# songhayeong/aes-fhe

Hardware: AMD Instinct MI355X
Metric: AES-128 blocks/sec (homomorphic full round) at N=2^16, L=30; 1/2/4/8 MI355X (higher is better)
Workload: dtype u64

## Files before the change

aes-fhe_amd/csrc/bconv_cols.h:

```cpp
#pragma once
#include "bconv_mfma.h"
#include "ntt256f.h"

namespace aesfhe {

__device__ __forceinline__ void cols256_stages_store(double (&x)[16], double q, double qi, bool big, const double* tg,
                                                     const double* tws, double* s, u64* out, int b, int cl, int c) {
#pragma unroll
    for (int st = 0; st < 4; st++) {
        const int m = 1 << st, hh = 8 >> st;
        if (big && st == 2) {
#pragma unroll
            for (int a = 0; a < 16; a++) x[a] = fred(x[a], q, qi);
        }
#pragma unroll
        for (int a = 0; a < 16; a++) {
            if (a & hh) continue;
            const int ti = m + (a >> (4 - st));
            ct_f(x[a], x[a + hh], tg[ti], q, qi);
        }
    }
#pragma unroll
    for (int a = 0; a < 16; a++) s[(a * 16 + b) * kPadF + cl] = x[a];
    __syncthreads();
// ... 6 lines not shown
        if (big && (st & 1) == 0) {
#pragma unroll
            for (int bb = 0; bb < 16; bb++) x[bb] = fred(x[bb], q, qi);
        }
#pragma unroll
        for (int bb = 0; bb < 16; bb++) {
            if (bb & hh) continue;
            ct_f(x[bb], x[bb + hh], tws[m + ap * (m >> 4) + (bb >> (8 - st))], q, qi);
        }
    }
#pragma unroll
    for (int bb = 0; bb < 16; bb++) st_d(&out[(ap * 16 + bb) * 256 + c], x[bb]);
}

template <int NSTEP, bool YIN, bool VC = false, int PF = 1, int TT = 4, int LT = 2, int MODE = 0>
__global__ __launch_bounds__(256, TT == 4 ? 2 : 3) void k_bconv_cols(BconvArgs a, Tabs T, int ntile) {
    static_assert(TT == 4 || TT == 2, "4 or 2 targets per workgroup");
    static_assert(LT == 1 || LT == 2, "1 or 2 LDS tiles");
    __shared__ double s[LT][256 * kPadF];
    __shared__ double tws[TT][256];
    const int tid = threadIdx.x, lane = tid & 63, w = tid >> 6, c = lane & 31, h = lane >> 5;
    const int cl = tid & 15, b = tid >> 4;
    const int id = blockIdx.x, x8 = id & 7, j = id >> 3;
    const int tile = j % ntile, u = (j / ntile) * 8 + x8;
    const int bx = u & 15, z = u >> 4, zb = z / a.nc, zc = z - zb * a.nc;
    const int logN = T.logN;
    const u64* src = a.src + (long)zb * a.sbs + (long)zc * a.scs;
    u64* dst = a.dst + (long)zb * a.dbs + (long)zc * a.dcs;
    auto limb_of = [&](int tau) { return tau < a.skip0 ? tau : tau + a.skipn; };
    auto pid_of = [&](int tl) { return tl <= a.tl_l ? tl : a.Lp1 + tl - a.tl_l - 1; };
    const int tau0 = TT * tile;
    const int nlive = min(TT, a.nt - tau0);
#pragma unroll
    for (int m = 0; m < TT; m++)
        if (m < nlive) tws[m][tid] = T.psid[((long)pid_of(limb_of(tau0 + m)) << logN) + tid];
    bc_v4i af[NSTEP];
    {
        const int row = lane & 31, ta = row >> 3, pb = (row & 3) + 4 * ((row >> 2) & 1);
        const int tau = tau0 + ta;
        const bc_v4i* ap =
            (const bc_v4i*)(a.tab + ((long)(ta < TT && tau < a.nt ? pid_of(limb_of(tau)) : 0) * 8 + pb) * kBconvKT + 16 * h);
#pragma unroll
        for (int st = 0; st < NSTEP; st++) af[st] = ap[2 * st];
    }
    const u64* sp[NSTEP][2];
    double sq[NSTEP][2], sf[NSTEP][2];
#pragma unroll
    for (int st = 0; st < NSTEP; st++)
#pragma unroll
        for (int uu = 0; uu < 2; uu++) {
            const int sl = 4 * st + 2 * h + uu;
            const int i = sl < a.ns ? sl : 0;
            sp[st][uu] = src + ((long)i << logN) + bx * 16 + (c & 15);
            if (!YIN) {
                const int pid = i < a.s_nq ? a.s_q0 + i : a.s_p0 + i - a.s_nq;
                sq[st][uu] = (double)a.qall[pid];
                sf[st][uu] = a.sinvf[i];
            }
        }
    double xv[TT][16];
    double eq[TT], eqi[TT], ew32[TT], ef32[TT], ecr[TT];
#pragma unroll
    for (int m = 0; m < TT; m++) {
        const int pid = tau0 + m < a.nt ? pid_of(limb_of(tau0 + m)) : 0;
        const double* pc = a.pc + 4 * pid;
        eq[m] = pc[0], eqi[m] = pc[1], ew32[m] = pc[2], ef32[m] = pc[3], ecr[m] = a.corr[pid];
    }
    double ev[VC ? 4 * NSTEP : 1];
#pragma unroll
    for (int sl = 0; sl < (VC ? 4 * NSTEP : 0); sl++) ev[sl] = a.einv[sl];
    u64 raw[PF + 1][NSTEP][2][2];
    auto load = [&](u64 (&r)[NSTEP][2][2], int ar) {
#pragma unroll
        for (int st = 0; st < NSTEP; st++)
#pragma unroll
            for (int uu = 0; uu < 2; uu++)
#pragma unroll
                for (int g = 0; g < 2; g++) r[st][uu][g] = sp[st][uu][(16 * ar + 4 * w + 2 * g + (c >> 4)) * 256];
    };
#pragma unroll
    for (int p = 0; p < PF; p++) load(raw[p], p);
#pragma unroll
    for (int ar = 0; ar < 16; ar++) {
        if (ar + PF < 16) load(raw[(ar + PF) % (PF + 1)], ar + PF);
        bc_v4i bf[2][NSTEP];
        double ys[2][NSTEP][2];
#pragma unroll
        for (int st = 0; st < NSTEP; st++)
#pragma unroll
            for (int uu = 0; uu < 2; uu++)
#pragma unroll
                for (int g = 0; g < 2; g++) {
                    u64 yb = PF ? raw[ar % (PF + 1)][st][uu][g] : sp[st][uu][(16 * ar + 4 * w + 2 * g + (c >> 4)) * 256];
                    if (!YIN) {
                        const double q = sq[st][uu], f = sf[st][uu];
                        double y = fmul_rem(u2d(yb), tw_w(f, q), f, q);
                        y = y < 0.0 ? y + q : y;
                        yb = (u64)__double_as_longlong(y + 4503599627370496.0) & 0xFFFFFFFFFFFFFULL;
                    }
                    if (VC) ys[g][st][uu] = u2d(yb);
                    bf[g][st][2 * uu] = (int)(unsigned)yb ^ (int)0x80808080;
                    bf[g][st][2 * uu + 1] = (int)(unsigned)(yb >> 32) ^ (int)0x80808080;
                }
        if constexpr (VC) {
            double yl[NSTEP][2][2];
#pragma unroll
            for (int st = 0; st < NSTEP; st++)
#pragma unroll
                for (int uu = 0; uu < 2; uu++) swap_halves(ys[0][st][uu], ys[1][st][uu], yl[st][uu][0], yl[st][uu][1]);
            double sum = 0.0;
#pragma unroll
            for (int st = 0; st < NSTEP; st++)
#pragma unroll
                for (int hh = 0; hh < 2; hh++)
#pragma unroll
                    for (int uu = 0; uu < 2; uu++) {
                        const int sl = 4 * st + 2 * hh + uu;
                        sum = sum + yl[st][uu][hh] * ev[sl];
                    }
            const int vown = (int)__builtin_rint(sum);
            const auto pr = __builtin_amdgcn_permlane32_swap((unsigned)vown, (unsigned)vown, false, false);
            const int voth = (int)(h ? pr[0] : pr[1]);
#pragma unroll
            for (int st = 0; st < NSTEP; st++)
#pragma unroll
                for (int uu = 0; uu < 2; uu++)
                    if (4 * st + 2 * h + uu == a.ns) {
#pragma unroll
                        for (int g = 0; g < 2; g++) {
                            bf[g][st][2 * uu] = ((g == h ? vown : voth) & 0xff) ^ (int)0x80808080;
                            bf[g][st][2 * uu + 1] = (int)0x80808080;
                        }
                    }
        }
        if constexpr (MODE == 2) {
#pragma unroll
            for (int m = 0; m < TT; m++) xv[m][ar] = (double)(bf[0][0][0] & 0xffffff) + (double)(bf[1][NSTEP - 1][3] & 0xff);
            continue;
        }
        bc_v16i acc[2];
#pragma unroll
        for (int g = 0; g < 2; g++) {
            acc[g] = bc_v16i{};
#pragma unroll
            for (int st = 0; st < NSTEP; st++) acc[g] = __builtin_amdgcn_mfma_i32_32x32x32_i8(af[st], bf[g][st], acc[g], 0, 0, 0);
        }
#pragma unroll
        for (int m = 0; m < TT; m++) {
            if (m >= nlive) break;
            double part[2];
#pragma unroll
            for (int g = 0; g < 2; g++) {
                const int p01 = acc[g][4 * m] + acc[g][4 * m + 1] * 256, p23 = acc[g][4 * m + 2] + acc[g][4 * m + 3] * 256;
                part[g] = __builtin_fma((double)p23, 65536.0, (double)p01);
            }
            double lo, hi;
            swap_halves(part[0], part[1], lo, hi);
            xv[m][ar] = fred(lo + fmul_rem(hi, ew32[m], ef32[m], eq[m]) + ecr[m], eq[m], eqi[m]);
        }
    }
    __syncthreads();
    if constexpr (MODE == 1) {
#pragma unroll
        for (int m = 0; m < TT; m++) {
            if (m >= nlive) break;
            u64* o = dst + ((long)limb_of(tau0 + m) << logN);
#pragma unroll
            for (int ar = 0; ar < 16; ar++) st_d(&o[(ar * 16 + b) * 256 + bx * 16 + cl], xv[m][ar]);
        }
        return;
    }
#pragma unroll
    for (int m = 0; m < TT; m++) {
        if (m >= nlive) break;
        if (LT == 1 && m > 0) __syncthreads();
        const int tl = limb_of(tau0 + m), pid = pid_of(tl);
        const double q = (double)T.q[pid], qi = T.qinv[pid];
        cols256_stages_store(xv[m], q, qi, q >= kBigPrime, T.psid + ((long)pid << logN), tws[m], s[m % LT],
                             dst + ((long)tl << logN), b, cl, bx * 16 + cl);
    }
}

}
```

aes-fhe_amd/csrc/bconv_mfma.h:

```cpp
#pragma once
#include "kernels.h"
#include "basis_tables.h"

namespace aesfhe {

typedef int bc_v4i __attribute__((ext_vector_type(4)));
typedef int bc_v16i __attribute__((ext_vector_type(16)));

struct BconvArgs {
    const u64* src;
    long sbs, scs;
    u64* dst;
    long dbs, dcs;
    int nc;
    int ns;
    int s_nq, s_q0, s_p0;
    const double* sinvf;
    const double* einv;
    int nt, skip0, skipn, tl_l, Lp1;
    const int8_t* tab;
    const double* corr;
    const double* pc;
    const u64* qall;
    const double* qinvall;
    int tiles_per_group;
};

__device__ __forceinline__ void swap_halves(double x, double y, double& xo, double& yo) {
    const u64 a = (u64)__double_as_longlong(x), b = (u64)__double_as_longlong(y);
    const auto lo = __builtin_amdgcn_permlane32_swap((unsigned)a, (unsigned)b, false, false);
    const auto hi = __builtin_amdgcn_permlane32_swap((unsigned)(a >> 32), (unsigned)(b >> 32), false, false);
    xo = __longlong_as_double((long long)(((u64)(unsigned)hi[0] << 32) | (unsigned)lo[0]));
    yo = __longlong_as_double((long long)(((u64)(unsigned)hi[1] << 32) | (unsigned)lo[1]));
}

template <int NSTEP, bool VC>
__global__ __launch_bounds__(256, 3) void k_bconv_mfma(BconvArgs a, int logN) {
    const int lane = threadIdx.x & 63, w = threadIdx.x >> 6;
    const int c = lane & 31, h = lane >> 5;
    const int z = blockIdx.z, zb = z / a.nc, zc = z - zb * a.nc;
    const long kb = (long)blockIdx.x * 256 + w * 64;
    const u64* src = a.src + (long)zb * a.sbs + (long)zc * a.scs;
    bc_v4i bf[2][NSTEP];
    double ys[2][2 * NSTEP];
#pragma unroll
    for (int s = 0; s < NSTEP; s++) {
#pragma unroll
        for (int u = 0; u < 2; u++) {
            const int sl = 4 * s + 2 * h + u;
            const bool live = sl < a.ns;
            const int i = live ? sl : 0;
            const int pid = i < a.s_nq ? a.s_q0 + i : a.s_p0 + i - a.s_nq;
            const double q = (double)a.qall[pid];
            const double f = a.sinvf[i], wv = tw_w(f, q);
            const u64* sp = src + ((long)i << logN) + kb + c;
#pragma unroll
            for (int g = 0; g < 2; g++) {
                double y = fmul_rem(u2d(sp[32 * g]), wv, f, q);
                y = y < 0.0 ? y + q : y;
                ys[g][2 * s + u] = live ? y : 0.0;
                const u64 yb = live ? ((u64)__double_as_longlong(y + 4503599627370496.0) & 0xFFFFFFFFFFFFFULL) : 0;
                bf[g][s][2 * u] = (int)(unsigned)yb ^ (int)0x80808080;
                bf[g][s][2 * u + 1] = (int)(unsigned)(yb >> 32) ^ (int)0x80808080;
            }
        }
    }
    if constexpr (VC) {
#pragma unroll
        for (int g = 0; g < 2; g++) {
            double other[2 * NSTEP];
#pragma unroll
// ... 93 lines not shown
```

aes-fhe_amd/csrc/engine.hip:

```cpp
#include <hip/hip_runtime.h>

#include <algorithm>
#include <atomic>
#include <cstdarg>
#include <cstdlib>
#include <cstdio>
#include <cstring>
#include <map>
#include <unordered_map>
#include <memory>
#include <mutex>
#include <string>
#include <vector>

#include "../../include/aesfhe.h"
#include "kernels_ops.h"
#include "ntt256f.h"
#include "ks_fused.h"
#include "bconv_mfma.h"
#include "bconv_cols.h"
#include "basis_tables.h"
#include "bsgs_plan.h"
#include "operands.h"
#include "arena.h"
// ... 399 lines not shown
    o.ptr = v.zero ? nullptr : v.d;
    o.bs = bcast_stride(v.B, v.bs, outB);
    o.ps = v.ps;
    o.np = v.np;
    o.bmask = (v.B > 1 && v.B < outB) ? v.B - 1 : -1;
    return o;
}

static Out out_of(aesfhe_ct* c) {
    Out o;
    o.ptr = c->d;
    o.ps = (long)(c->level + 1) * c->eng->N;
    o.bs = (long)c->np * o.ps;
    return o;
}

static View view_of(const CtPtr& c) { return view_of(c.get()); }
static Out out_of(const CtPtr& c) { return out_of(c.get()); }

static dim3 ew_grid(aesfhe_engine* e, int y, int z) { return dim3(e->N / 256, y, z); }

template <int R1>
static void ntt_fwd_t(aesfhe_engine* e, Span src, Span dst, int total) {
    constexpr int CW = (kTile / R1) < kC2 ? (kTile / R1) : kC2;
    constexpr int RW = (kTile / kC2) < R1 ? (kTile / kC2) : R1;
    Tabs T = e->tabs();
    const double by = 8.0 * e->N * (double)total;
    {
        ProfScope ps(e, FAM_NTT, by, "ntt_generic");
        hipLaunchKernelGGL(k_ntt_fwd_cols<R1>, dim3(kC2 / CW, total), dim3(256), 0, e->stream, src, dst, T);
    }
    {
        ProfScope ps(e, FAM_NTT, by, "ntt_generic");
        hipLaunchKernelGGL(k_ntt_fwd_rows<R1>, dim3(R1 / RW, total), dim3(256), 0, e->stream, dst, T);
    }
}
template <int R1>
static void ntt_inv_t(aesfhe_engine* e, Span src, Span dst, int total) {
    constexpr int CW = (kTile / R1) < kC2 ? (kTile / R1) : kC2;
    constexpr int RW = (kTile / kC2) < R1 ? (kTile / kC2) : R1;
    Tabs T = e->tabs();
    const double by = 8.0 * e->N * (double)total;
    {
        ProfScope ps(e, FAM_NTT, by, "ntt_generic");
        hipLaunchKernelGGL(k_ntt_inv_rows<R1>, dim3(R1 / RW, total), dim3(256), 0, e->stream, src, dst, T);
    }
    {
        ProfScope ps(e, FAM_NTT, by, "ntt_generic");
        hipLaunchKernelGGL(k_ntt_inv_cols<R1>, dim3(kC2 / CW, total), dim3(256), 0, e->stream, dst, T);
    }
}

template <int R>
static void ntt256(aesfhe_engine* e, Span src, Span dst, int total, bool inverse, const double* lf = nullptr) {
    Tabs T = e->tabs();
    const double by = 8.0 * e->N * (double)total;
    {
        ProfScope ps(e, FAM_NTT, by, inverse ? "ntt_inv_rows" : "ntt_fwd_cols");
        if (!inverse) hipLaunchKernelGGL(k_nttf_fwd_cols<R>, dim3(16, total), dim3(256), 0, e->stream, src, dst, T);
        else hipLaunchKernelGGL((k_nttf_inv_rows<R, false>), dim3(R / 16, total), dim3(256), 0, e->stream, src, dst, T, Span{}, (const u64*)nullptr);
    }
    ProfScope ps(e, FAM_NTT, by, inverse ? "ntt_inv_cols" : "ntt_fwd_rows");
    if (!inverse) hipLaunchKernelGGL((k_nttf_fwd_rows_t<false, R>), dim3(R / 16, total), dim3(256), 0, e->stream, dst, T, RowFin{});
    else if (lf) hipLaunchKernelGGL((k_nttf_inv_cols<R, true>), dim3(16, total), dim3(256), 0, e->stream, dst, T, lf);
    else hipLaunchKernelGGL((k_nttf_inv_cols<R, false>), dim3(16, total), dim3(256), 0, e->stream, dst, T, (const double*)nullptr);
}

static bool fused_ntt(const aesfhe_engine* e) { return e->logN == 16 || e->logN == 17; }

static void intt_prod(aesfhe_engine* e, Span a, Span b, Span dst, int total, const u64* fac, const double* lf = nullptr) {
    if (total <= 0) return;
    Tabs T = e->tabs();
    const double by = 8.0 * e->N * (double)total;
    {
        ProfScope ps(e, FAM_NTT, 2.0 * by, "ntt_inv_rows_prod");
        if (e->logN == 16) {
            if (fac) hipLaunchKernelGGL((k_nttf_inv_rows<256, true, true>), dim3(16, total), dim3(256), 0, e->stream, a, dst, T, b, fac);
            else hipLaunchKernelGGL((k_nttf_inv_rows<256, true, false>), dim3(16, total), dim3(256), 0, e->stream, a, dst, T, b, fac);
        } else {
            if (fac) hipLaunchKernelGGL((k_nttf_inv_rows<512, true, true>), dim3(32, total), dim3(256), 0, e->stream, a, dst, T, b, fac);
            else hipLaunchKernelGGL((k_nttf_inv_rows<512, true, false>), dim3(32, total), dim3(256), 0, e->stream, a, dst, T, b, fac);
        }
    }
    ProfScope ps(e, FAM_NTT, by, "ntt_inv_cols");
    if (e->logN == 16) {
        if (lf) hipLaunchKernelGGL((k_nttf_inv_cols<256, true>), dim3(16, total), dim3(256), 0, e->stream, dst, T, lf);
        else hipLaunchKernelGGL((k_nttf_inv_cols<256, false>), dim3(16, total), dim3(256), 0, e->stream, dst, T, lf);
    } else {
        if (lf) throw_err(AESFHE_EUNSUPPORTED, "per-limb INTT factors at N = 2^17");
        hipLaunchKernelGGL((k_nttf_inv_cols<512, false>), dim3(16, total), dim3(256), 0, e->stream, dst, T, lf);
    }
    HIPC(hipGetLastError());
}

static void ntt_fwd_cols(aesfhe_engine* e, Span src, Span dst, int total) {
    if (e->logN == 16) hipLaunchKernelGGL(k_nttf_fwd_cols<256>, dim3(16, total), dim3(256), 0, e->stream, src, dst, e->tabs());
    else hipLaunchKernelGGL(k_nttf_fwd_cols<512>, dim3(16, total), dim3(256), 0, e->stream, src, dst, e->tabs());
}
static void ntt_fwd_cols(aesfhe_engine* e, Span sp, int total) { ntt_fwd_cols(e, sp, sp, total); }

static void ntt(aesfhe_engine* e, Span src, Span dst, int total, bool inverse) {
    if (total <= 0) return;
    if (e->logN == 16 || e->logN == 17) {
        if (e->logN == 16) ntt256<256>(e, src, dst, total, inverse);
        else ntt256<512>(e, src, dst, total, inverse);
        HIPC(hipGetLastError());
        return;
    }
    switch (e->logN) {
#define CASE(LG, R)                                                        \
    case LG:                                                               \
        if (inverse) ntt_inv_t<R>(e, src, dst, total);                     \
        else ntt_fwd_t<R>(e, src, dst, total);                             \
        break;
        CASE(10, 4)
        CASE(11, 8)
        CASE(12, 16)
        CASE(13, 32)
        CASE(14, 64)
        CASE(15, 128)
        CASE(16, 256)
        CASE(17, 512)
#undef CASE
        default:
            throw_err(AESFHE_EUNSUPPORTED, "log_n %d not supported by the HIP NTT", e->logN);
    }
    HIPC(hipGetLastError());
}

static Span span_s(u64* base, long pstride, int nl, int nq, int qpid0, int spid0) {
    Span s;
    s.base = base;
    s.pstride = pstride;
    s.nl = nl;
    s.nq = nq;
    s.qpid0 = qpid0;
    s.spid0 = spid0;
    return s;
}


static void build_tables(aesfhe_engine* e) {
    const int N = e->N, np = e->np, L = e->L, K = e->K, Lp1 = e->Lp1;
// ... 1204 lines not shown
    const dim3 g(N / 256, groups, nz);
#define BCV(S, V) hipLaunchKernelGGL((k_bconv_mfma<S, V>), g, dim3(256), 0, e->stream, a, e->logN)
    switch (nstep * 2 + (vc ? 1 : 0)) {
        case 2: BCV(1, false); break;
        case 3: BCV(1, true); break;
        case 4: BCV(2, false); break;
        case 5: BCV(2, true); break;
        case 6: BCV(3, false); break;
        case 7: BCV(3, true); break;
        case 8: BCV(4, false); break;
        default: BCV(4, true); break;
    }
#undef BCV
    HIPC(hipGetLastError());
}

static bool fused_bconv(const aesfhe_engine* e) { return e->logN == 16; }

static BconvArgs modup_args(const aesfhe_engine* e, const u64* dc, int l, int j, u64* dst, bool ysrc) {
    const int lo = j * e->A, alpha = std::min(lo + e->A, l + 1) - lo, ne = l + 1 + e->K;
    const size_t set = (size_t)j * e->A + (alpha - 1);
    BconvArgs a{};
    a.src = dc + (long)lo * e->N;
    a.sbs = (long)(l + 1) * e->N;
    a.dst = dst;
    a.dbs = (long)ne * e->N;
    a.nc = 1;
    a.ns = alpha;
    a.s_nq = alpha;
    a.s_q0 = lo;
    a.sinvf = ysrc ? nullptr : e->mu_hatinvf + set * e->A;
    a.nt = ne - alpha;
    a.skip0 = lo;
    a.skipn = alpha;
    a.tl_l = l;
    a.Lp1 = e->Lp1;
    a.tab = e->bc_mu_tab + set * e->np * 8 * kBconvKT;
    a.corr = e->bc_mu_corr + set * e->np;
    a.pc = e->bc_pc;
    a.qall = e->q;
    a.qinvall = e->qinv;
    return a;
}

static MdTabs md_tabs(const aesfhe_engine* e, int l, int r) {
    if (r < 0 || r > kMdrMaxR || e->K + r > kMdrMaxE || l - r < 0) throw_err(AESFHE_EARG, "bad combined rescale depth %d", r);
    const size_t cell = md_cell(e->Lp1, r, l), ce = cell * kMdrMaxE, cl = cell * e->Lp1;
    const MdTabs& b = e->md;
    return {b.invf + ce, b.ninvf + ce, b.einv + ce, b.tab + cl * kBconvRow, b.corr + cl,
            b.dinv + cl, b.dinvf + cl, b.hatf + cl * kMdrMaxE, b.dmodf + cl};
}

static BconvArgs moddown_args(const aesfhe_engine* e, const MdTabs& t, const u64* acc, long abs_, long acs, int l, int r,
                              u64* dst, bool ysrc) {
    const int lk = l - r;
    const long kN = (long)(lk + 1) * e->N;
    BconvArgs a{};
    a.src = acc + kN;
    a.sbs = abs_;
    a.scs = acs;
    a.dst = dst;
    a.dbs = 2 * kN;
    a.dcs = kN;
    a.nc = 2;
    a.ns = e->K + r;
    a.s_nq = r;
    a.s_q0 = lk + 1;
    a.s_p0 = e->Lp1;
    a.sinvf = ysrc ? nullptr : t.invf;
    a.einv = t.einv;
    a.nt = lk + 1;
    a.skip0 = lk + 1;
    a.skipn = 0;
    a.tl_l = lk;
    a.Lp1 = e->Lp1;
    a.tab = t.tab;
    a.corr = t.corr;
    a.pc = e->bc_pc;
    a.qall = e->q;
    a.qinvall = e->qinv;
    return a;
}

template <bool VC>
static void launch_bconv_cols_t(aesfhe_engine* e, const BconvArgs& a, int nz, int nslots) {
    const int nstep = (nslots + 3) / 4, ntile = (a.nt + 3) / 4;
    if (e->logN != 16 || nstep < 1 || nstep > 4 || ntile < 1 || (16 * nz) % 8)
        throw_err(AESFHE_EUNSUPPORTED, "fused base conversion of %d slots to %d targets", nslots, a.nt);
    if (!a.src || !a.dst || !a.tab || !a.corr || !a.pc || (VC && !a.einv))
        throw_err(AESFHE_EUNSUPPORTED, "fused base conversion with a missing table");
    const dim3 g((unsigned)(16 * nz * ntile));
    const Tabs T = e->tabs();
#define BCC(S) hipLaunchKernelGGL((k_bconv_cols<S, true, VC, 1>), g, dim3(256), 0, e->stream, a, T, ntile)
    switch (nstep) {
        case 1: BCC(1); break;
        case 2: BCC(2); break;
        case 3: BCC(3); break;
        default: BCC(4); break;
    }
#undef BCC
    HIPC(hipGetLastError());
}
static void launch_bconv_cols(aesfhe_engine* e, const BconvArgs& a, int nz) { launch_bconv_cols_t<false>(e, a, nz, a.ns); }

static std::vector<unsigned short> bsgs_block_order(int logN, const std::vector<u64>& gal) {
    std::vector<unsigned short> ord;
    if (!aesfhe::bsgs_block_order(logN, std::vector<uint64_t>(gal.begin(), gal.end()), ord))
        throw_err(AESFHE_EUNSUPPORTED, "bsgs block order is not a permutation");
    return ord;
}

static int ks_beta(const aesfhe_engine* e, int l) {
    const int beta = (l + 1 + e->A - 1) / e->A;
    if (beta > 12) throw_err(AESFHE_EUNSUPPORTED, "more than 12 key-switch digits");
    return beta;
}
static void check_key_digits(aesfhe_engine* e, const aesfhe_key* k, int l) {
    if (k && k->ndig > 0 && ks_beta(e, l) > k->ndig)
        throw_err(AESFHE_ELEVEL, "key trimmed to %d digits cannot switch at level %d (%d digits)", k->ndig, l, ks_beta(e, l));
}

static void ks_modup(aesfhe_engine* e, const u64* d, long dbs, int B, int l, u64* ext, bool cols_only = false,
                     const Opnd* pa = nullptr, const Opnd* pb = nullptr, const u64* fac = nullptr) {
    const int N = e->N, K = e->K, ne = l + 1 + K;
    const long lN = (long)(l + 1) * N, neN = (long)ne * N;
    const int beta = ks_beta(e, l);
    Tmp dc(e, (size_t)B * lN);
    const bool fcols = fused_bconv(e);
    const double* lf = fcols ? e->mu_nhatf + (size_t)l * e->Lp1 : nullptr;
    Span sdc = span_s(dc.p, lN, l + 1, l + 1, 0, e->Lp1);
    if (pa) {
        Span sa = span_s((u64*)pa->ptr + pa->ps, pa->bs, l + 1, l + 1, 0, e->Lp1);
        Span sb = span_s((u64*)pb->ptr + pb->ps, pb->bs, l + 1, l + 1, 0, e->Lp1);
        sa.pmask = pa->bmask;
        sb.pmask = pb->bmask;
        intt_prod(e, sa, sb, sdc, B * (l + 1), fac, lf);
    } else {
        Span sd = span_s((u64*)d, dbs, l + 1, l + 1, 0, e->Lp1);
        if (lf) ntt256<256>(e, sd, sdc, B * (l + 1), true, lf);
        else ntt(e, sd, sdc, B * (l + 1), true);
    }
    Tmp mu;
    bool any_wide = false;
    for (int j = 0; j < beta; j++) any_wide |= std::min((j + 1) * e->A, l + 1) - j * e->A > 1;
    if (cols_only && any_wide && !fcols) mu = Tmp(e, (size_t)B * neN);
    for (int j = 0; j < beta; j++) {
        const int A = e->A, lo = j * A, hi = std::min(lo + A, l + 1), alpha = hi - lo;
        u64* exj = ext + (size_t)j * B * neN;
        u64* muj = mu ? mu.p : exj;
        if (cols_only && alpha == 1) {
            const SpreadSrc ss{(const u64*)dc.p + (long)lo * N, lN, 0, 0, 0.0};
            auto kern = N == 65536 ? k_nttf_fwd_cols_spread<256, 3> : k_nttf_fwd_cols_spread<512, 3>;
            auto cols = [&](Span sp, int total) {
                ProfScope ps(e, FAM_NTT, 8.0 * N * (double)total, "ntt_fwd_cols_spread");
                hipLaunchKernelGGL(kern, dim3(16, total), dim3(256), 0, e->stream, ss, sp, e->tabs());
            };
            if (lo > 0) cols(span_s(exj, neN, lo, lo, 0, e->Lp1), B * lo);
            cols(span_s(exj + (long)hi * N, neN, ne - hi, (l + 1) - hi, hi, e->Lp1), B * (ne - hi));
            HIPC(hipGetLastError());
            continue;
        }
        if (fcols) {
            const BconvArgs a = modup_args(e, dc.p, l, j, exj, true);
            {
                ProfScope ps(e, FAM_KS, 8.0 * N * (double)B * ne, "modup_cols");
                launch_bconv_cols(e, a, B);
            }
            if (!cols_only) {
                auto rows = [&](long off, int n, int nq, int p0, int total) {
                    ProfScope ps(e, FAM_NTT, 8.0 * N * (double)total, "ntt_fwd_rows");
                    hipLaunchKernelGGL((k_nttf_fwd_rows_t<false, 256>), dim3(16, total), dim3(256), 0, e->stream,
                                       span_s(exj + off, neN, n, nq, p0, e->Lp1), e->tabs(), RowFin{});
                    HIPC(hipGetLastError());
                };
                if (lo > 0) rows(0, lo, lo, 0, B * lo);
                rows((long)hi * N, ne - hi, (l + 1) - hi, hi, B * (ne - hi));
            }
            continue;
        }
        {
            ProfScope ps(e, FAM_KS, 8.0 * N * (double)B * ne, "modup");
            launch_bconv(e, modup_args(e, dc.p, l, j, muj, false), B, alpha, false);
        }
        auto fwd = [&](long off, int n, int nq, int p0, int total) {
            Span sp = span_s(exj + off, neN, n, nq, p0, e->Lp1);
            if (!cols_only) return ntt(e, sp, sp, total, false);
            ProfScope ps(e, FAM_NTT, 8.0 * N * (double)total, "ntt_fwd_cols");
            ntt_fwd_cols(e, span_s(muj + off, neN, n, nq, p0, e->Lp1), sp, total);
        };
        if (lo > 0) fwd(0, lo, lo, 0, B * lo);
        fwd((long)hi * N, ne - hi, (l + 1) - hi, hi, B * (ne - hi));
    }
}

static void ks_inner_acc(aesfhe_engine* e, const u64* d, long dbs, const u64* ext, int B, int l,
                         const aesfhe_key* k, Opnd addend, bool pmod, u64* acc, bool ext_cols, bool accum = false) {
    const int N = e->N, K = e->K, ne = l + 1 + K;
    const long neN = (long)ne * N;
    const int beta = ks_beta(e, l);
    check_key_digits(e, k, l);
    const double* pm = pmod ? (const double*)e->pmodf : (const double*)nullptr;
    if (ext_cols) {
        const int nown = std::min(l + 1, beta * e->A);
        const double opw = (double)nown + (pmod && addend.ptr ? (double)addend.np * (l + 1) : 0.0);
        ProfScope ps(e, FAM_KS, 8.0 * N * ((double)B * (beta * ne - nown + opw) + (double)ne * (2.0 * beta + 2.0 * B * (accum ? 2 : 1))), "ks_rows_acc.ks");
        const int R = N / 256, blocks = 8 * B * (ne * (R / 8) / 8);
        const Opnd none{nullptr, 0, 0, 0};
        auto kern = R == 256 ? k_nttf_rows_ks<1, 256, false> : k_nttf_rows_ks<1, 512, false>;
        hipLaunchKernelGGL(kern, dim3(blocks), dim3(256), 0, e->stream, d, dbs, ext, neN, (long)B * neN, (const u64*)k->d, 2L * e->np * N, (long)e->np * N, acc, 2 * neN, neN, B, beta, e->A, l, ne, e->tabs(), addend, pm, (int)accum, none, (const u64*)nullptr, none, 0, ne, KsFin{});
    } else {
        ProfScope ps(e, FAM_KS, 8.0 * N * (double)ne * (beta * B + 2.0 * beta + 2.0 * B * (accum ? 2 : 1)), "ks_inner");
        auto inner = beta <= 4 ? k_ks_inner_all<4> : beta <= 8 ? k_ks_inner_all<8> : k_ks_inner_all<12>;
        hipLaunchKernelGGL(inner, dim3(N / 256, ne, 1), dim3(256), 0, e->stream, d, dbs, ext, neN, (long)B * neN, (const u64*)k->d, 2L * e->np * N, (long)e->np * N, acc, 2 * neN, neN, B, beta, e->A, l, e->q, e->qinv, e->Lp1, addend, pm, e->logN, (int)accum);
    }
    HIPC(hipGetLastError());
}

static void moddown_conv(aesfhe_engine* e, const MdTabs& t, u64* acc, long abs_, long acs, int B, int l, int r, u64* conv,
                         bool rows_done) {
    const int N = e->N, K = e->K, lk = l - r;
    const long kN = (long)(lk + 1) * N;
    {
        Span ssp = span_s(acc + kN, acs, K + r, r, lk + 1, e->Lp1);
        const int total = B * 2 * (K + r);
        if (rows_done) {
            ProfScope ps(e, FAM_NTT, 8.0 * N * (double)total, "ntt_inv_cols");
            if (N == 65536) hipLaunchKernelGGL((k_nttf_inv_cols<256, false>), dim3(16, total), dim3(256), 0, e->stream, ssp, e->tabs(), (const double*)nullptr);
            else hipLaunchKernelGGL((k_nttf_inv_cols<512, false>), dim3(16, total), dim3(256), 0, e->stream, ssp, e->tabs(), (const double*)nullptr);
            HIPC(hipGetLastError());
        } else {
            ntt(e, ssp, ssp, total, true);
        }
    }
    {
        ProfScope ps(e, FAM_KS, 8.0 * N * (double)B * 2 * (K + r + lk + 1), "moddown");
        if (K + r < 1 || K + r > 16) throw_err(AESFHE_EUNSUPPORTED, "ModDown source width outside 1..16");
        if (K + r + 1 <= 16)
            launch_bconv(e, moddown_args(e, t, acc, abs_, acs, l, r, conv, false), B * 2, K + r + 1, true);
        else
            AESFHE_DISPATCH16(K + r, launch_moddown, dim3(N / 512, bconv_groups(N, B * 2, lk + 1), B * 2), e->stream, (const u64*)acc, abs_, acs, l, r, conv, 2 * kN, kN,
                              t.invf, t.hatf, t.einv, t.dmodf, e->Lp1, e->q, e->qinv, e->logN, kMdrMaxE);
    }
    HIPC(hipGetLastError());
}

static bool moddown_cols_ok(const aesfhe_engine* e, int r) { return fused_bconv(e) && e->K + r + 1 <= 16; }
static void moddown_conv_cols(aesfhe_engine* e, const MdTabs& t, u64* acc, long abs_, long acs, int B, int l, int r,
                              u64* conv2, bool rows_done) {
    const int N = e->N, K = e->K, lk = l - r;
    {
        Span ssp = span_s(acc + (long)(lk + 1) * N, acs, K + r, r, lk + 1, e->Lp1);
        const int total = B * 2 * (K + r);
        if (!rows_done) {
            ProfScope ps(e, FAM_NTT, 8.0 * N * (double)total, "ntt_inv_rows");
            hipLaunchKernelGGL((k_nttf_inv_rows<256, false>), dim3(16, total), dim3(256), 0, e->stream, ssp, ssp, e->tabs(),
                               Span{}, (const u64*)nullptr);
            HIPC(hipGetLastError());
        }
        ProfScope ps(e, FAM_NTT, 8.0 * N * (double)total, "ntt_inv_cols");
        hipLaunchKernelGGL((k_nttf_inv_cols<256, true>), dim3(16, total), dim3(256), 0, e->stream, ssp, e->tabs(), t.ninvf);
        HIPC(hipGetLastError());
    }
    ProfScope ps(e, FAM_KS, 8.0 * N * (double)B * 2 * (K + r + lk + 1), "moddown_cols");
    launch_bconv_cols_t<true>(e, moddown_args(e, t, acc, abs_, acs, l, r, conv2, true), 2 * B, K + r + 1);
}

struct Conv2 {
    Tmp conv, buf;
};
template <typename F>
static Conv2 moddown_conv2(aesfhe_engine* e, const MdTabs& t, u64* acc, long abs_, long acs, int B, int l, int r,
                           bool rows_done, F converted) {
    const int lk = l - r, total = B * 2 * (lk + 1);
    const long kN = (long)(lk + 1) * e->N;
    Conv2 c;
    if (moddown_cols_ok(e, r)) {
        c.buf = Tmp(e, (size_t)B * 2 * kN);
        moddown_conv_cols(e, t, acc, abs_, acs, B, l, r, c.buf.p, rows_done);
        converted();
        return c;
    }
    c.conv = Tmp(e, (size_t)B * 2 * kN);
    moddown_conv(e, t, acc, abs_, acs, B, l, r, c.conv.p, rows_done);
    converted();
    c.buf = Tmp(e, (size_t)B * 2 * kN);
    ProfScope ps(e, FAM_NTT, 8.0 * e->N * (double)total, "ntt_fwd_cols");
    ntt_fwd_cols(e, span_s(c.conv.p, kN, lk + 1, lk + 1, 0, e->Lp1), span_s(c.buf.p, kN, lk + 1, lk + 1, 0, e->Lp1), total);
    return c;
}

static void moddown_acc(aesfhe_engine* e, u64* acc, int B, int l, int r, Opnd fin_add, aesfhe_ct* o) {
    const int N = e->N, ne = l + 1 + e->K, lk = l - r;
    const long neN = (long)ne * N, kN = (long)(lk + 1) * N;
    const MdTabs t = md_tabs(e, l, r);
    if (fused_ntt(e)) {
        const Conv2 c = moddown_conv2(e, t, acc, 2 * neN, neN, B, l, r, false, [] {});
        const int total = B * 2 * (lk + 1);
        RowFin f{(const u64*)acc, 2 * neN, neN, Opnd2{fin_add.ptr, fin_add.bs, fin_add.ps, fin_add.np}, o->d,
                 2 * kN, kN, t.dinvf, lk + 1};
        ProfScope ps(e, FAM_NTT, 8.0 * N * (double)total * (3.0 + (fin_add.ptr ? 1.0 : 0.0)), "ntt_fwd_rows_fin");
        auto kern = N == 65536 ? k_nttf_fwd_rows_t<true, 256> : k_nttf_fwd_rows_t<true, 512>;
        hipLaunchKernelGGL(kern, dim3(N / 4096, total), dim3(256), 0, e->stream, span_s(c.buf.p, kN, lk + 1, lk + 1, 0, e->Lp1),
                           e->tabs(), f);
        HIPC(hipGetLastError());
        return;
    }
    Tmp conv(e, (size_t)B * 2 * kN);
    moddown_conv(e, t, acc, 2 * neN, neN, B, l, r, conv.p, false);
    Span sc = span_s(conv.p, kN, lk + 1, lk + 1, 0, e->Lp1);
    ntt(e, sc, sc, B * 2 * (lk + 1), false);
    ProfScope psf(e, FAM_KS, 8.0 * N * (double)B * 2 * (lk + 1) * 4, "moddown_finish");
    hipLaunchKernelGGL(k_moddown_finish, dim3(N / 256, lk + 1, B * 2), dim3(256), 0, e->stream, (const u64*)acc, 2 * neN, neN, (const u64*)conv.p, 2 * kN, kN, fin_add, out_of(o), e->q, t.dinv, t.dinvf, e->logN);
    HIPC(hipGetLastError());
}

template <int R>
static decltype(&k_nttf_rows_ks_p<R, false, 1>) ks_rows_kernel(bool prod, bool fin) {
// ... 1090 lines not shown
```

aes-fhe_amd/csrc/ntt256f.h:

```cpp
#pragma once
#include <type_traits>

#include "kernels.h"

namespace aesfhe {


__device__ __forceinline__ void ct_f(double& x, double& y, double w, double q, double qi) {
    const double v = fmul_remq(y, w, qi, q);
    const double t = x;
    x = t + v;
    y = t - v;
}
template <bool FOLD>
__device__ __forceinline__ void gs_f(double& x, double& y, double w, double q, double qi) {
    const double s = x + y, d = x - y;
    x = FOLD ? fred(s, q, qi) : s;
    y = fmul_remq(d, w, qi, q);
}
__device__ __forceinline__ double tw_row(const double* W, int idx, double rw, double q, double qi) {
    return fmul_remq(W[idx], rw, qi, q);
}
__device__ __forceinline__ double ld_d(const u64* p) { return __longlong_as_double((long long)*p); }
__device__ __forceinline__ void st_d(u64* p, double v) { __builtin_nontemporal_store((u64)__double_as_longlong(v), p); }
// ... 265 lines not shown
                s[row_tile_idx(e)] = u2d(gb[e]);
            }
        }
    }
    wave_sync_lds();
    double* sr = s + rl * 16 * kPadF;
    const int ap = b;
    double x[16];
#pragma unroll
    for (int bb = 0; bb < 16; bb++) x[bb] = sr[ap * kPadF + bb];
    const double* R = T.irtwd + (long)pid * RR * 8 + row * 8;
    auto stages_lo = [&](auto fold) {
#pragma unroll
        for (int st = 0; st < 4; st++) {
            const int t = 1 << st, ml = 128 / t, nj = 8 / t;
            const double rw = R[7 - st];
#pragma unroll
            for (int j = 0; j < nj; j++) {
                const double w = tw_row(W, RR * ml + ap * nj + j, rw, q, qi);
#pragma unroll
                for (int k = 0; k < t; k++)
                    gs_f<decltype(fold)::value>(x[j * 2 * t + k], x[j * 2 * t + k + t], w, q, qi);
            }
        }
    };
    if (big) stages_lo(std::true_type{});
    else stages_lo(std::false_type{});
#pragma unroll
    for (int bb = 0; bb < 16; bb++) sr[ap * kPadF + bb] = x[bb];
    wave_sync_lds();
#pragma unroll
    for (int a = 0; a < 16; a++) x[a] = sr[a * kPadF + b];
    auto stages_hi = [&](auto fold) {
#pragma unroll
        for (int st = 4; st < 8; st++) {
            const int t = 1 << st, ta = t >> 4, ml = 128 / t;
            const double rw = R[7 - st];
#pragma unroll
            for (int j = 0; j < ml; j++) {
                const double w = tw_row(W, RR * ml + j, rw, q, qi);
#pragma unroll
                for (int k = 0; k < ta; k++)
                    gs_f<decltype(fold)::value>(x[j * 2 * ta + k], x[j * 2 * ta + k + ta], w, q, qi);
            }
        }
    };
    if (big) stages_hi(std::true_type{});
    else stages_hi(std::false_type{});
    u64* op = out + (long)row * 256;
#pragma unroll
    for (int a = 0; a < 16; a++) st_d(&op[a * 16 + b], x[a]);
}

template <int R = 256, bool LF = false>
__global__ __launch_bounds__(256) void k_nttf_inv_cols(Span dst, Tabs T, const double* __restrict__ lf) {
    static_assert(R == 256 || R == 512, "rows of 256: N = 2^16 or 2^17");
    constexpr int H = R / 256;
    __shared__ double s[256 * kPadF];
    __shared__ double tws[R];
    int pid;
    u64* io = span_ptr(dst, blockIdx.y, T.logN, T.Lp1, pid);
    const int tid = threadIdx.x, cl = tid & 15, b = tid >> 4;
    const int c = blockIdx.x * 16 + cl;
    const double q = (double)T.q[pid], qi = T.qinv[pid];
    const bool big = q >= kBigPrime;
    const double* tg = T.ipsid + ((long)pid << T.logN);
#pragma unroll
    for (int h = 0; h < H; h++) tws[tid + 256 * h] = tg[tid + 256 * h];
    const int ap = b;
    double x[16 * H];
#pragma unroll
    for (int h = 0; h < H; h++)
#pragma unroll
        for (int bb = 0; bb < 16; bb++) x[16 * h + bb] = fred(ld_d(&io[(h * 256 + ap * 16 + bb) * 256 + c]), q, qi);
    __syncthreads();
#pragma unroll
    for (int h = 0; h < H; h++) {
        double* xh = x + 16 * h;
        const int mul = H == 1 ? 1 : 2 + h;
        auto stages_lo = [&](auto fold) {
#pragma unroll
            for (int st = 0; st < 4; st++) {
                const int tr = 1 << st;
                const int base = (128 / tr) * mul + ap * (8 / tr);
#pragma unroll
                for (int bb = 0; bb < 16; bb++) {
                    if (bb & tr) continue;
                    gs_f<decltype(fold)::value>(xh[bb], xh[bb + tr], tws[base + (bb >> (st + 1))], q, qi);
                }
            }
        };
        if (big) stages_lo(std::true_type{});
        else stages_lo(std::false_type{});
        if (h > 0) __syncthreads();
#pragma unroll
        for (int bb = 0; bb < 16; bb++) s[(ap * 16 + bb) * kPadF + cl] = xh[bb];
        __syncthreads();
#pragma unroll
        for (int a = 0; a < 16; a++) xh[a] = s[(a * 16 + b) * kPadF + cl];
        auto stages_hi = [&](auto fold) {
#pragma unroll
            for (int st = 4; st < 8; st++) {
                const int tr = 1 << st, ta = tr >> 4;
                const int base = (128 / tr) * mul;
#pragma unroll
                for (int a = 0; a < 16; a++) {
                    if (a & ta) continue;
                    const int ti = base + (a >> (st - 3));
                    gs_f<decltype(fold)::value>(xh[a], xh[a + ta], tg[ti], q, qi);
                }
            }
        };
        if (big) stages_hi(std::true_type{});
        else stages_hi(std::false_type{});
    }
    if (H == 2) {
        const double w = tg[1];
#pragma unroll
        for (int a = 0; a < 16; a++) {
            x[a] = fred(x[a], q, qi);
            x[16 + a] = fred(x[16 + a], q, qi);
            gs_f<false>(x[a], x[16 + a], w, q, qi);
        }
    }
    const double nif = LF ? lf[blockIdx.y % dst.nl] : T.ninvf[pid];
    const double ni = LF ? tw_w(nif, q) : (double)T.ninv[pid];
#pragma unroll
    for (int h = 0; h < H; h++)
#pragma unroll
        for (int a = 0; a < 16; a++) {
            const double r = fred(x[16 * h + a], q, qi);
            __builtin_nontemporal_store(fcanon(fmul_rem(r, ni, nif, q), q, qi), &io[(h * 256 + a * 16 + b) * 256 + c]);
        }
}


}
```

Measured before the change: 285,800.

## Fuse ModDown v-estimate into looped inverse NTT and pre-bias bconv inputs

Adds a specialized inverse-NTT kernel for ModDown that loops over all dropped limbs of a polynomial per workgroup, accumulating the v correction sum in registers and writing a separate v plane. The base-conversion kernel then reads v from that plane instead of recomputing it per tile with cross-lane swaps. INTT outputs are also pre-XORed with the int8 bias so the bconv inner loop skips that XOR. The trade is fewer parallel workgroups, since the grid now runs over polynomials rather than limbs, plus an extra temporary buffer and a serial per-limb loop.

After: 286,000 (median of 2 runs). About the same (+0.1%).

```diff
diff --git a/aes-fhe_amd/csrc/bconv_cols.h b/aes-fhe_amd/csrc/bconv_cols.h
--- a/aes-fhe_amd/csrc/bconv_cols.h
+++ b/aes-fhe_amd/csrc/bconv_cols.h
@@ -82,6 +82,7 @@
             const int sl = 4 * st + 2 * h + uu;
             const int i = sl < a.ns ? sl : 0;
             sp[st][uu] = src + ((long)i << logN) + bx * 16 + (c & 15);
+            if (VC && sl == a.ns) sp[st][uu] = a.v + (long)zb * a.vbs + (long)zc * a.vcs + bx * 16 + (c & 15);
             if (!YIN) {
                 const int pid = i < a.s_nq ? a.s_q0 + i : a.s_p0 + i - a.s_nq;
                 sq[st][uu] = (double)a.qall[pid];
@@ -96,9 +97,6 @@
         const double* pc = a.pc + 4 * pid;
         eq[m] = pc[0], eqi[m] = pc[1], ew32[m] = pc[2], ef32[m] = pc[3], ecr[m] = a.corr[pid];
     }
-    double ev[VC ? 4 * NSTEP : 1];
-#pragma unroll
-    for (int sl = 0; sl < (VC ? 4 * NSTEP : 0); sl++) ev[sl] = a.einv[sl];
     u64 raw[PF + 1][NSTEP][2][2];
     auto load = [&](u64 (&r)[NSTEP][2][2], int ar) {
 #pragma unroll
@@ -114,7 +112,6 @@
     for (int ar = 0; ar < 16; ar++) {
         if (ar + PF < 16) load(raw[(ar + PF) % (PF + 1)], ar + PF);
         bc_v4i bf[2][NSTEP];
-        double ys[2][NSTEP][2];
 #pragma unroll
         for (int st = 0; st < NSTEP; st++)
 #pragma unroll
@@ -126,43 +123,11 @@
                         const double q = sq[st][uu], f = sf[st][uu];
                         double y = fmul_rem(u2d(yb), tw_w(f, q), f, q);
                         y = y < 0.0 ? y + q : y;
-                        yb = (u64)__double_as_longlong(y + 4503599627370496.0) & 0xFFFFFFFFFFFFFULL;
+                        yb = ((u64)__double_as_longlong(y + 4503599627370496.0) & 0xFFFFFFFFFFFFFULL) ^ kBconvBias;
                     }
-                    if (VC) ys[g][st][uu] = u2d(yb);
-                    bf[g][st][2 * uu] = (int)(unsigned)yb ^ (int)0x80808080;
-                    bf[g][st][2 * uu + 1] = (int)(unsigned)(yb >> 32) ^ (int)0x80808080;
+                    bf[g][st][2 * uu] = (int)(unsigned)yb;
+                    bf[g][st][2 * uu + 1] = (int)(unsigned)(yb >> 32);
                 }
-        if constexpr (VC) {
-            double yl[NSTEP][2][2];
-#pragma unroll
-            for (int st = 0; st < NSTEP; st++)
-#pragma unroll
-                for (int uu = 0; uu < 2; uu++) swap_halves(ys[0][st][uu], ys[1][st][uu], yl[st][uu][0], yl[st][uu][1]);
-            double sum = 0.0;
-#pragma unroll
-            for (int st = 0; st < NSTEP; st++)
-#pragma unroll
-                for (int hh = 0; hh < 2; hh++)
-#pragma unroll
-                    for (int uu = 0; uu < 2; uu++) {
-                        const int sl = 4 * st + 2 * hh + uu;
-                        sum = sum + yl[st][uu][hh] * ev[sl];
-                    }
-            const int vown = (int)__builtin_rint(sum);
-            const auto pr = __builtin_amdgcn_permlane32_swap((unsigned)vown, (unsigned)vown, false, false);
-            const int voth = (int)(h ? pr[0] : pr[1]);
-#pragma unroll
-            for (int st = 0; st < NSTEP; st++)
-#pragma unroll
-                for (int uu = 0; uu < 2; uu++)
-                    if (4 * st + 2 * h + uu == a.ns) {
-#pragma unroll
-                        for (int g = 0; g < 2; g++) {
-                            bf[g][st][2 * uu] = ((g == h ? vown : voth) & 0xff) ^ (int)0x80808080;
-                            bf[g][st][2 * uu + 1] = (int)0x80808080;
-                        }
-                    }
-        }
         if constexpr (MODE == 2) {
 #pragma unroll
             for (int m = 0; m < TT; m++) xv[m][ar] = (double)(bf[0][0][0] & 0xffffff) + (double)(bf[1][NSTEP - 1][3] & 0xff);
diff --git a/aes-fhe_amd/csrc/bconv_mfma.h b/aes-fhe_amd/csrc/bconv_mfma.h
--- a/aes-fhe_amd/csrc/bconv_mfma.h
+++ b/aes-fhe_amd/csrc/bconv_mfma.h
@@ -17,6 +17,8 @@
     int s_nq, s_q0, s_p0;
     const double* sinvf;
     const double* einv;
+    const u64* v;
+    long vbs, vcs;
     int nt, skip0, skipn, tl_l, Lp1;
     const int8_t* tab;
     const double* corr;
diff --git a/aes-fhe_amd/csrc/engine.hip b/aes-fhe_amd/csrc/engine.hip
--- a/aes-fhe_amd/csrc/engine.hip
+++ b/aes-fhe_amd/csrc/engine.hip
@@ -475,7 +475,7 @@
 }
 
 template <int R>
-static void ntt256(aesfhe_engine* e, Span src, Span dst, int total, bool inverse, const double* lf = nullptr) {
+static void ntt256(aesfhe_engine* e, Span src, Span dst, int total, bool inverse, const double* lf = nullptr, int plain_from = 0) {
     Tabs T = e->tabs();
     const double by = 8.0 * e->N * (double)total;
     {
@@ -485,13 +485,14 @@
     }
     ProfScope ps(e, FAM_NTT, by, inverse ? "ntt_inv_cols" : "ntt_fwd_rows");
     if (!inverse) hipLaunchKernelGGL((k_nttf_fwd_rows_t<false, R>), dim3(R / 16, total), dim3(256), 0, e->stream, dst, T, RowFin{});
-    else if (lf) hipLaunchKernelGGL((k_nttf_inv_cols<R, true>), dim3(16, total), dim3(256), 0, e->stream, dst, T, lf);
-    else hipLaunchKernelGGL((k_nttf_inv_cols<R, false>), dim3(16, total), dim3(256), 0, e->stream, dst, T, (const double*)nullptr);
+    else if (lf) hipLaunchKernelGGL((k_nttf_inv_cols<R, true>), dim3(16, total), dim3(256), 0, e->stream, dst, T, lf, plain_from);
+    else hipLaunchKernelGGL((k_nttf_inv_cols<R, false>), dim3(16, total), dim3(256), 0, e->stream, dst, T, (const double*)nullptr, 0);
 }
 
 static bool fused_ntt(const aesfhe_engine* e) { return e->logN == 16 || e->logN == 17; }
 
-static void intt_prod(aesfhe_engine* e, Span a, Span b, Span dst, int total, const u64* fac, const double* lf = nullptr) {
+static void intt_prod(aesfhe_engine* e, Span a, Span b, Span dst, int total, const u64* fac, const double* lf = nullptr,
+                      int plain_from = 0) {
     if (total <= 0) return;
     Tabs T = e->tabs();
     const double by = 8.0 * e->N * (double)total;
@@ -507,11 +508,11 @@
     }
     ProfScope ps(e, FAM_NTT, by, "ntt_inv_cols");
     if (e->logN == 16) {
-        if (lf) hipLaunchKernelGGL((k_nttf_inv_cols<256, true>), dim3(16, total), dim3(256), 0, e->stream, dst, T, lf);
-        else hipLaunchKernelGGL((k_nttf_inv_cols<256, false>), dim3(16, total), dim3(256), 0, e->stream, dst, T, lf);
+        if (lf) hipLaunchKernelGGL((k_nttf_inv_cols<256, true>), dim3(16, total), dim3(256), 0, e->stream, dst, T, lf, plain_from);
+        else hipLaunchKernelGGL((k_nttf_inv_cols<256, false>), dim3(16, total), dim3(256), 0, e->stream, dst, T, lf, 0);
     } else {
         if (lf) throw_err(AESFHE_EUNSUPPORTED, "per-limb INTT factors at N = 2^17");
-        hipLaunchKernelGGL((k_nttf_inv_cols<512, false>), dim3(16, total), dim3(256), 0, e->stream, dst, T, lf);
+        hipLaunchKernelGGL((k_nttf_inv_cols<512, false>), dim3(16, total), dim3(256), 0, e->stream, dst, T, lf, 0);
     }
     HIPC(hipGetLastError());
 }
@@ -1822,7 +1823,7 @@
 }
 
 static BconvArgs moddown_args(const aesfhe_engine* e, const MdTabs& t, const u64* acc, long abs_, long acs, int l, int r,
-                              u64* dst, bool ysrc) {
+                              u64* dst, bool ysrc, const u64* vplane = nullptr) {
     const int lk = l - r;
     const long kN = (long)(lk + 1) * e->N;
     BconvArgs a{};
@@ -1839,6 +1840,9 @@
     a.s_p0 = e->Lp1;
     a.sinvf = ysrc ? nullptr : t.invf;
     a.einv = t.einv;
+    a.v = vplane;
+    a.vbs = 2L * e->N;
+    a.vcs = e->N;
     a.nt = lk + 1;
     a.skip0 = lk + 1;
     a.skipn = 0;
@@ -1857,7 +1861,7 @@
     const int nstep = (nslots + 3) / 4, ntile = (a.nt + 3) / 4;
     if (e->logN != 16 || nstep < 1 || nstep > 4 || ntile < 1 || (16 * nz) % 8)
         throw_err(AESFHE_EUNSUPPORTED, "fused base conversion of %d slots to %d targets", nslots, a.nt);
-    if (!a.src || !a.dst || !a.tab || !a.corr || !a.pc || (VC && !a.einv))
+    if (!a.src || !a.dst || !a.tab || !a.corr || !a.pc || (VC && !a.v))
         throw_err(AESFHE_EUNSUPPORTED, "fused base conversion with a missing table");
     const dim3 g((unsigned)(16 * nz * ntile));
     const Tabs T = e->tabs();
@@ -1898,16 +1902,17 @@
     Tmp dc(e, (size_t)B * lN);
     const bool fcols = fused_bconv(e);
     const double* lf = fcols ? e->mu_nhatf + (size_t)l * e->Lp1 : nullptr;
+    const int plain_from = !cols_only ? l + 1 : e->A == 1 ? 0 : l % e->A == 0 ? l : l + 1;
     Span sdc = span_s(dc.p, lN, l + 1, l + 1, 0, e->Lp1);
     if (pa) {
         Span sa = span_s((u64*)pa->ptr + pa->ps, pa->bs, l + 1, l + 1, 0, e->Lp1);
         Span sb = span_s((u64*)pb->ptr + pb->ps, pb->bs, l + 1, l + 1, 0, e->Lp1);
         sa.pmask = pa->bmask;
         sb.pmask = pb->bmask;
-        intt_prod(e, sa, sb, sdc, B * (l + 1), fac, lf);
+        intt_prod(e, sa, sb, sdc, B * (l + 1), fac, lf, plain_from);
     } else {
         Span sd = span_s((u64*)d, dbs, l + 1, l + 1, 0, e->Lp1);
-        if (lf) ntt256<256>(e, sd, sdc, B * (l + 1), true, lf);
+        if (lf) ntt256<256>(e, sd, sdc, B * (l + 1), true, lf, plain_from);
         else ntt(e, sd, sdc, B * (l + 1), true);
     }
     Tmp mu;
@@ -1995,8 +2000,8 @@
         const int total = B * 2 * (K + r);
         if (rows_done) {
             ProfScope ps(e, FAM_NTT, 8.0 * N * (double)total, "ntt_inv_cols");
-            if (N == 65536) hipLaunchKernelGGL((k_nttf_inv_cols<256, false>), dim3(16, total), dim3(256), 0, e->stream, ssp, e->tabs(), (const double*)nullptr);
-            else hipLaunchKernelGGL((k_nttf_inv_cols<512, false>), dim3(16, total), dim3(256), 0, e->stream, ssp, e->tabs(), (const double*)nullptr);
+            if (N == 65536) hipLaunchKernelGGL((k_nttf_inv_cols<256, false>), dim3(16, total), dim3(256), 0, e->stream, ssp, e->tabs(), (const double*)nullptr, 0);
+            else hipLaunchKernelGGL((k_nttf_inv_cols<512, false>), dim3(16, total), dim3(256), 0, e->stream, ssp, e->tabs(), (const double*)nullptr, 0);
             HIPC(hipGetLastError());
         } else {
             ntt(e, ssp, ssp, total, true);
@@ -2018,6 +2023,8 @@
 static void moddown_conv_cols(aesfhe_engine* e, const MdTabs& t, u64* acc, long abs_, long acs, int B, int l, int r,
                               u64* conv2, bool rows_done) {
     const int N = e->N, K = e->K, lk = l - r;
+    if (abs_ != 2 * acs) throw_err(AESFHE_EARG, "ModDown accumulators are not [B][2] polynomials of one stride");
+    Tmp vplane(e, (size_t)B * 2 * N);
     {
         Span ssp = span_s(acc + (long)(lk + 1) * N, acs, K + r, r, lk + 1, e->Lp1);
         const int total = B * 2 * (K + r);
@@ -2027,12 +2034,13 @@
                                Span{}, (const u64*)nullptr);
             HIPC(hipGetLastError());
         }
-        ProfScope ps(e, FAM_NTT, 8.0 * N * (double)total, "ntt_inv_cols");
-        hipLaunchKernelGGL((k_nttf_inv_cols<256, true>), dim3(16, total), dim3(256), 0, e->stream, ssp, e->tabs(), t.ninvf);
+        ProfScope ps(e, FAM_NTT, 8.0 * N * (double)(total + 2 * B), "ntt_inv_cols");
+        hipLaunchKernelGGL((k_nttf_inv_cols<MdLoop>), dim3(16, 2 * B), dim3(256), 0, e->stream, ssp, e->tabs(), t.ninvf, t.einv,
+                           vplane.p, (long)N);
         HIPC(hipGetLastError());
     }
-    ProfScope ps(e, FAM_KS, 8.0 * N * (double)B * 2 * (K + r + lk + 1), "moddown_cols");
-    launch_bconv_cols_t<true>(e, moddown_args(e, t, acc, abs_, acs, l, r, conv2, true), 2 * B, K + r + 1);
+    ProfScope ps(e, FAM_KS, 8.0 * N * (double)B * 2 * (K + r + 1 + lk + 1), "moddown_cols");
+    launch_bconv_cols_t<true>(e, moddown_args(e, t, acc, abs_, acs, l, r, conv2, true, vplane.p), 2 * B, K + r + 1);
 }
 
 struct Conv2 {
diff --git a/aes-fhe_amd/csrc/ntt256f.h b/aes-fhe_amd/csrc/ntt256f.h
--- a/aes-fhe_amd/csrc/ntt256f.h
+++ b/aes-fhe_amd/csrc/ntt256f.h
@@ -341,8 +341,9 @@
     for (int a = 0; a < 16; a++) st_d(&op[a * 16 + b], x[a]);
 }
 
+constexpr u64 kBconvBias = 0x8080808080808080ULL;
 template <int R = 256, bool LF = false>
-__global__ __launch_bounds__(256) void k_nttf_inv_cols(Span dst, Tabs T, const double* __restrict__ lf) {
+__global__ __launch_bounds__(256) void k_nttf_inv_cols(Span dst, Tabs T, const double* __restrict__ lf, int plain_from) {
     static_assert(R == 256 || R == 512, "rows of 256: N = 2^16 or 2^17");
     constexpr int H = R / 256;
     __shared__ double s[256 * kPadF];
@@ -412,16 +413,100 @@
             gs_f<false>(x[a], x[16 + a], w, q, qi);
         }
     }
-    const double nif = LF ? lf[blockIdx.y % dst.nl] : T.ninvf[pid];
+    const int li = blockIdx.y % dst.nl;
+    const double nif = LF ? lf[li] : T.ninvf[pid];
     const double ni = LF ? tw_w(nif, q) : (double)T.ninv[pid];
+    const u64 bias = LF && li < plain_from ? kBconvBias : 0;
 #pragma unroll
     for (int h = 0; h < H; h++)
 #pragma unroll
         for (int a = 0; a < 16; a++) {
             const double r = fred(x[16 * h + a], q, qi);
-            __builtin_nontemporal_store(fcanon(fmul_rem(r, ni, nif, q), q, qi), &io[(h * 256 + a * 16 + b) * 256 + c]);
-        }
-}
-
-
-}
+            __builtin_nontemporal_store(fcanon(fmul_rem(r, ni, nif, q), q, qi) ^ bias, &io[(h * 256 + a * 16 + b) * 256 + c]);
+        }
+}
+
+struct MdLoop {};
+template <typename V>
+__device__ __forceinline__ V ld_tab(const V* p) {
+    return *(const __attribute__((address_space(4))) V*)p;
+}
+template <typename Form>
+__global__ __launch_bounds__(256, 4) void k_nttf_inv_cols(Span dst, Tabs T, const double* __restrict__ lf,
+                                                          const double* __restrict__ einv, u64* __restrict__ vp, long vs) {
+    static_assert(std::is_same<Form, MdLoop>::value, "the ModDown loop over a polynomial's dropped limbs");
+    __shared__ double tws[256];
+    __shared__ double s[256 * kPadF];
+    const int tid = threadIdx.x, cl = tid & 15, b = tid >> 4, ap = b;
+    const int c = blockIdx.x * 16 + cl;
+    u64* base = dst.base + (long)blockIdx.y * dst.pstride;
+    const unsigned ol = (ap * 4096 + c) * 8, os = (b * 256 + c) * 8;
+    typedef __attribute__((address_space(1))) char gchar;
+    typedef __attribute__((address_space(1))) u64 gu64;
+    auto at = [](const u64* p, unsigned byte_off) {
+        asm("" : "+s"(p));
+        return (gu64*)((gchar*)p + byte_off);
+    };
+    u64 raw[16];
+#pragma unroll
+    for (int bb = 0; bb < 16; bb++) raw[bb] = *at(base + bb * 256, ol);
+    double sum[16];
+#pragma unroll
+    for (int a = 0; a < 16; a++) sum[a] = 0.0;
+#pragma unroll 1
+    for (int j = 0; j < dst.nl; j++) {
+        const int pid = j < dst.nq ? dst.qpid0 + j : dst.spid0 + (j - dst.nq);
+        u64* io = base + ((long)j << 16);
+        const double q = (double)ld_tab(T.q + pid), qi = ld_tab(T.qinv + pid);
+        const double* tg = T.ipsid + ((long)pid << 16);
+        tws[tid] = tg[tid];
+        double x[16];
+#pragma unroll
+        for (int bb = 0; bb < 16; bb++) x[bb] = fred(__longlong_as_double((long long)raw[bb]), q, qi);
+        __syncthreads();
+#pragma unroll
+        for (int st = 0; st < 4; st++) {
+            const int tr = 1 << st;
+            const int tb = (128 / tr) + ap * (8 / tr);
+#pragma unroll
+            for (int bb = 0; bb < 16; bb++) {
+                if (bb & tr) continue;
+                gs_f<true>(x[bb], x[bb + tr], tws[tb + (bb >> (st + 1))], q, qi);
+            }
+        }
+#pragma unroll
+        for (int bb = 0; bb < 16; bb++) s[(ap * 16 + bb) * kPadF + cl] = x[bb];
+        __syncthreads();
+#pragma unroll
+        for (int a = 0; a < 16; a++) x[a] = s[(a * 16 + b) * kPadF + cl];
+#pragma unroll
+        for (int st = 4; st < 8; st++) {
+            const int tr = 1 << st, ta = tr >> 4;
+#pragma unroll
+            for (int a = 0; a < 16; a++) {
+                if (a & ta) continue;
+                gs_f<true>(x[a], x[a + ta], ld_tab(tg + (128 / tr) + (a >> (st - 3))), q, qi);
+            }
+        }
+        const double nif = ld_tab(lf + j), ni = tw_w(nif, q), ej = ld_tab(einv + j);
+        const bool more = j + 1 < dst.nl;
+#pragma unroll
+        for (int a = 0; a < 16; a++) {
+            double y = fred(fmul_rem(fred(x[a], q, qi), ni, nif, q), q, qi);
+            y = y < 0.0 ? y + q : y;
+            const u64 w = (u64)__double_as_longlong(y + 4503599627370496.0) & 0xFFFFFFFFFFFFFULL;
+            __builtin_nontemporal_store(w ^ kBconvBias, at(io + a * 4096, os));
+            sum[a] = sum[a] + y * ej;
+            raw[a] = more ? *at(io + 65536 + a * 256, ol) : 0;
+        }
+    }
+    u64* vo = vp + (long)blockIdx.y * vs;
+#pragma unroll
+    for (int a = 0; a < 16; a++) {
+        const int v = (int)__builtin_rint(sum[a]);
+        __builtin_nontemporal_store((u64)(unsigned)(v & 0xff) ^ kBconvBias, at(vo + a * 4096, os));
+    }
+}
+
+
+}
```
